# hpcaitech/Open-Sora

Measured on NVIDIA H100. Metric: denoise-steps/sec STDiT3-XL/2 64x32x32 bf16, higher is better.
Workload: dtype bf16

## Files before the change

### open-sora_b200/csrc/attn_sm90.cu

```cuda
#include <stdlib.h>

#include "common.cuh"
#include "stage.cuh"
#include "tiles.cuh"
#include "wgmma.cuh"

namespace osb {

constexpr int kAttnThreads = 256;
constexpr int kKeyBlock = 64;

template <int D>
struct FlashState {
  static constexpr int DP = HeadTileCfg<D>::DP;
  uint32_t q[DP / 16][4];
  float o[DP / 8][4];
  float m[2], l[2];
};

template <int D>
__device__ __forceinline__ void flash_load_q(FlashState<D>& f, uint32_t sq, uint32_t chunk_bytes) {
  using Cfg = HeadTileCfg<D>;
  const int lane = threadIdx.x & 31, warp = threadIdx.x >> 5;
  const int row = warp * 16 + (lane & 15);
#pragma unroll
  for (int kk = 0; kk < Cfg::DP / 16; ++kk)
    ldsm_x4(sq + tile_unit_off<Cfg::MAIN>(row, 2 * kk + (lane >> 4), chunk_bytes), f.q[kk][0], f.q[kk][1], f.q[kk][2], f.q[kk][3]);
#pragma unroll
  for (int j = 0; j < Cfg::DP / 8; ++j) f.o[j][0] = f.o[j][1] = f.o[j][2] = f.o[j][3] = 0.f;
  f.m[0] = f.m[1] = -INFINITY;
  f.l[0] = f.l[1] = 0.f;
}

template <int D, bool kBias = false>
__device__ __forceinline__ void flash_block(FlashState<D>& f, uint32_t sk, uint32_t sv, uint32_t chunk_bytes, int krow0,
                                            int n16, int key0, const int (&lo)[2], const int (&hi)[2], float sc,
                                            const float* bias = nullptr, int boff0 = 0, int boff1 = 0, float bscale = 0.f) {
  using Cfg = HeadTileCfg<D>;
  constexpr int NB = kKeyBlock / 8;
  const int lane = threadIdx.x & 31;
  float s[NB][4];
#pragma unroll
  for (int g = 0; g < kKeyBlock / 16; ++g) {
    s[2 * g][0] = s[2 * g][1] = s[2 * g][2] = s[2 * g][3] = 0.f;
    s[2 * g + 1][0] = s[2 * g + 1][1] = s[2 * g + 1][2] = s[2 * g + 1][3] = 0.f;
    if (g >= n16) continue;
    const int krow = krow0 + g * 16 + (lane & 7) + ((lane >> 4) << 3);
#pragma unroll
    for (int kk = 0; kk < Cfg::DP / 16; ++kk) {
      uint32_t b0, b1, b2, b3;
      ldsm_x4(sk + tile_unit_off<Cfg::MAIN>(krow, 2 * kk + ((lane >> 3) & 1), chunk_bytes), b0, b1, b2, b3);
      mma_bf16_16816(s[2 * g], f.q[kk], b0, b1);
      mma_bf16_16816(s[2 * g + 1], f.q[kk], b2, b3);
// ... 40 lines not shown
    if (g >= n16) continue;
    const uint32_t a[4] = {pack_bf16x2(s[2 * g][0], s[2 * g][1]), pack_bf16x2(s[2 * g][2], s[2 * g][3]),
                           pack_bf16x2(s[2 * g + 1][0], s[2 * g + 1][1]), pack_bf16x2(s[2 * g + 1][2], s[2 * g + 1][3])};
    const int vrow = krow0 + g * 16 + (lane & 7) + (((lane >> 3) & 1) << 3);
#pragma unroll
    for (int dg = 0; dg < Cfg::DP / 16; ++dg) {
      uint32_t b0, b1, b2, b3;
      ldsm_x4_t(sv + tile_unit_off<Cfg::MAIN>(vrow, 2 * dg + (lane >> 4), chunk_bytes), b0, b1, b2, b3);
      mma_bf16_16816(f.o[2 * dg], a, b0, b1);
      mma_bf16_16816(f.o[2 * dg + 1], a, b2, b3);
    }
  }
}

template <int D>
__device__ __forceinline__ void flash_store(FlashState<D>& f, __nv_bfloat16* dst0, __nv_bfloat16* dst1) {
  const int lane = threadIdx.x & 31;
  float inv[2];
#pragma unroll
  for (int i = 0; i < 2; ++i) {
    float l = f.l[i];
    l += __shfl_xor_sync(0xffffffffu, l, 1);
    l += __shfl_xor_sync(0xffffffffu, l, 2);
    inv[i] = l > 0.f ? 1.0f / l : 0.f;
  }
#pragma unroll
  for (int j = 0; j < D / 8; ++j) {
    const int c = 8 * j + 2 * (lane & 3);
    if (dst0) *reinterpret_cast<uint32_t*>(dst0 + c) = pack_bf16x2(f.o[j][0] * inv[0], f.o[j][1] * inv[0]);
    if (dst1) *reinterpret_cast<uint32_t*>(dst1 + c) = pack_bf16x2(f.o[j][2] * inv[1], f.o[j][3] * inv[1]);
  }
}

struct TileAttnParams {
  const uint8_t* q; const uint8_t* k; const uint8_t* v;
  int64_t q_head_stride, kv_head_stride;
  int32_t q_tile_bytes, kv_tile_bytes;
  int64_t items;
  float scale_log2;
  TileSets ts;
};

template <int D>
struct TileAttnSmem {
  static constexpr int kSlot = 128 * HeadTileCfg<D>::ROW_BYTES;
  static constexpr int kStages = D == 128 ? 2 : (D == 72 ? 4 : 5);
  static constexpr int kData = 2 * kSlot + kStages * 2 * kSlot;
  static constexpr int kBytes = 1024 + kData + 8 * (4 + 2 * kStages);
  static_assert(kBytes <= 227 * 1024 && 2 * kBytes > 228 * 1024, "one resident CTA per SM");
};

constexpr int kTileAttnThreads = 384;

template <int D>
__global__ void __launch_bounds__(kTileAttnThreads, 1) attn_tiles_kernel(const TileAttnParams p) {
  using Cfg = HeadTileCfg<D>;
  using Sm = TileAttnSmem<D>;
  constexpr int MAIN = Cfg::MAIN, TAIL = Cfg::TAIL, STAGES = Sm::kStages;
  extern __shared__ uint8_t smem_raw[];
  const uint32_t base = (smem_u32(smem_raw) + 1023u) & ~1023u;
  auto sQ = [&](int b) { return base + (uint32_t)(b * Sm::kSlot); };
  auto sK = [&](int s) { return base + (uint32_t)((2 + 2 * s) * Sm::kSlot); };
  auto sV = [&](int s) { return sK(s) + (uint32_t)Sm::kSlot; };
  const uint32_t bar = base + (uint32_t)Sm::kData;
  auto q_full = [&](int b) { return bar + 8u * b; };
  auto q_empty = [&](int b) { return bar + 16u + 8u * b; };
  auto full_bar = [&](int s) { return bar + 32u + 8u * s; };
  auto empty_bar = [&](int s) { return bar + 32u + 8u * (STAGES + s); };

  const int wg = threadIdx.x >> 7, tid_wg = threadIdx.x & 127;
  const int64_t begin = (int64_t)blockIdx.x * p.items / gridDim.x, end = (int64_t)(blockIdx.x + 1) * p.items / gridDim.x;
  const TileSets& ts = p.ts;
  const int tps = ts.qmap.tps;

  {
    uint4* z = reinterpret_cast<uint4*>(smem_raw + (base - smem_u32(smem_raw)));
    for (int i = threadIdx.x; i < Sm::kData / 16; i += kTileAttnThreads) z[i] = make_uint4(0, 0, 0, 0);
  }
  fence_proxy_async_smem();
  if (threadIdx.x == 0) {
    for (int b = 0; b < 2; ++b) { mbar_init(q_full(b), 1); mbar_init(q_empty(b), 2); }
    for (int s = 0; s < STAGES; ++s) { mbar_init(full_bar(s), 1); mbar_init(empty_bar(s), 2); }
    fence_barrier_init();
  }
  __syncthreads();
  pdl_wait();

  if (wg == 0) {
    asm volatile("setmaxnreg.dec.sync.aligned.u32 40;\n" ::: "memory");
    if (tid_wg == 0) {
      uint32_t kv_it = 0;
      for (int64_t it = begin; it < end; ++it) {
        const uint32_t n = (uint32_t)(it - begin);
        const int64_t hs = it / tps, head = hs / ts.num_sets, set = hs - head * ts.num_sets;
        const int qs = n & 1;
        mbar_wait_notrace(q_empty(qs), ((n >> 1) & 1u) ^ 1u);
        mbar_expect_tx(q_full(qs), (uint32_t)p.q_tile_bytes);
        bulk_load_1d(sQ(qs), p.q + head * p.q_head_stride + (it - head * ts.num_sets * tps) * p.q_tile_bytes,
                     (uint32_t)p.q_tile_bytes, q_full(qs));
        const int nkt = (tile_set_keys(ts, set) + ts.BK - 1) / ts.BK;
        if (it > begin && (it - 1) / tps == hs && nkt <= STAGES) continue;
        const int64_t off = head * p.kv_head_stride + set * ts.nkb * (int64_t)p.kv_tile_bytes;
        for (int t = 0; t < nkt; ++t, ++kv_it) {
          const int s = (int)(kv_it % STAGES);
          mbar_wait_notrace(empty_bar(s), ((kv_it / STAGES) & 1u) ^ 1u);
          mbar_expect_tx(full_bar(s), 2u * (uint32_t)p.kv_tile_bytes);
          bulk_load_1d(sK(s), p.k + off + (int64_t)t * p.kv_tile_bytes, (uint32_t)p.kv_tile_bytes, full_bar(s));
          bulk_load_1d(sV(s), p.v + off + (int64_t)t * p.kv_tile_bytes, (uint32_t)p.kv_tile_bytes, full_bar(s));
        }
      }
      pdl_launch_dependents();
    }
    return;
  }

  asm volatile("setmaxnreg.inc.sync.aligned.u32 232;\n" ::: "memory");
  const int cw = wg - 1;
  const int lane = tid_wg & 31, quad = lane & 3;
  const int r_loc = cw * 64 + (tid_wg >> 5) * 16 + (lane >> 2);
  const float sc = p.scale_log2;
  float s[64], o[MAIN][32], ot[TAIL ? 8 : 1];
#pragma unroll
  for (int i = 0; i < 64; ++i) s[i] = 0.f;
  uint32_t kv_it = 0, kv0 = 0;
  for (int64_t it = begin; it < end; ++it) {
    const uint32_t n = (uint32_t)(it - begin);
    const int64_t hs = it / tps, head = hs / ts.num_sets, set = hs - head * ts.num_sets;
    const int qt = (int)(it - hs * tps), qs = n & 1;
    const int keys = tile_set_keys(ts, set);
    const int nkt = (keys + ts.BK - 1) / ts.BK;
    if (!(it > begin && (it - 1) / tps == hs && nkt <= STAGES)) { kv0 = kv_it; kv_it += nkt; }
    const bool keep = it + 1 < end && (it + 1) / tps == hs && nkt <= STAGES;

    int64_t seq[2];
    int pos[2], lo[2], hi[2];
    bool valid[2];
#pragma unroll
    for (int hh = 0; hh < 2; ++hh) tile_query_row(ts, set, qt, keys, r_loc + 8 * hh, seq[hh], pos[hh], valid[hh], lo[hh], hi[hh]);
#pragma unroll
    for (int c = 0; c < MAIN; ++c)
#pragma unroll
      for (int i = 0; i < 32; ++i) o[c][i] = 0.f;
#pragma unroll
    for (int i = 0; i < (TAIL ? 8 : 1); ++i) ot[i] = 0.f;
    float m[2] = {-INFINITY, -INFINITY}, l[2] = {0.f, 0.f};

    const uint32_t q_chunk = (uint32_t)ts.qmap.TR * 128u, kv_chunk = (uint32_t)ts.BK * 128u;
    const uint32_t qa = sQ(qs) + (uint32_t)(cw * 64 * 128), qa_tail = sQ(qs) + MAIN * q_chunk + (uint32_t)(cw * 8 * 256);
    mbar_wait_notrace(q_full(qs), (n >> 1) & 1u);
    for (int t = 0; t < nkt; ++t) {
      const uint32_t u = kv0 + (uint32_t)t;
      const int st = (int)(u % STAGES);
      mbar_wait_notrace(full_bar(st), (u / STAGES) & 1u);
      const uint32_t ka = sK(st), va = sV(st);
      wgmma_fence_regs(s);
      wgmma_fence();
#pragma unroll
      for (int c = 0; c < MAIN; ++c)
#pragma unroll
        for (int k = 0; k < 4; ++k)
          Wgmma<128>::mma(s, make_sw128_kmajor_desc(qa + c * q_chunk + 32u * k),
                          make_sw128_kmajor_desc(ka + c * kv_chunk + 32u * k), (c | k) ? 1u : 0u);
      if constexpr (TAIL != 0)
        Wgmma<128>::mma(s, make_noswizzle_desc(qa_tail, 128u, 256u), make_noswizzle_desc(ka + MAIN * kv_chunk, 128u, 256u), 1u);
      wgmma_commit();
      wgmma_wait<0>();
      wgmma_fence_regs(s);
      if (t == nkt - 1 && tid_wg == 0) mbar_arrive(q_empty(qs));
      const int slot0 = t * ts.BK;
      const int n16 = ((keys - slot0 < ts.BK ? keys - slot0 : ts.BK) + 15) >> 4;
      float mx[2] = {-INFINITY, -INFINITY};
#pragma unroll
      for (int i = 0; i < 64; ++i) {
        const int hh = (i >> 1) & 1;
        const int col = 8 * (i >> 2) + 2 * quad + (i & 1), key = slot0 + col;
        if (col >= ts.BK || key < lo[hh] || key >= hi[hh]) s[i] = -INFINITY;
        mx[hh] = fmaxf(mx[hh], s[i]);
      }
      float alpha[2], ms[2];
#pragma unroll
      for (int hh = 0; hh < 2; ++hh) {
        mx[hh] = fmaxf(mx[hh], __shfl_xor_sync(0xffffffffu, mx[hh], 1));
        mx[hh] = fmaxf(mx[hh], __shfl_xor_sync(0xffffffffu, mx[hh], 2));
        const float mn = fmaxf(m[hh], mx[hh]);
        alpha[hh] = (mn == -INFINITY) ? 1.f : fast_exp2((m[hh] - mn) * sc);
        ms[hh] = (mn == -INFINITY) ? 0.f : mn * sc;
        m[hh] = mn;
        l[hh] *= alpha[hh];
      }
#pragma unroll
      for (int c = 0; c < MAIN; ++c)
#pragma unroll
        for (int i = 0; i < 32; ++i) o[c][i] *= alpha[(i >> 1) & 1];
      if constexpr (TAIL != 0) {
#pragma unroll
        for (int i = 0; i < 8; ++i) ot[i] *= alpha[(i >> 1) & 1];
      }
      uint32_t pa[8][4];
#pragma unroll
      for (int i = 0; i < 64; ++i) {
        s[i] = (i >> 3) < n16 ? fast_exp2(fmaf(s[i], sc, -ms[(i >> 1) & 1])) : 0.f;
        l[(i >> 1) & 1] += s[i];
      }
#pragma unroll
      for (int g = 0; g < 8; ++g) {
        pa[g][0] = pack_bf16x2(s[8 * g + 0], s[8 * g + 1]);
        pa[g][1] = pack_bf16x2(s[8 * g + 2], s[8 * g + 3]);
        pa[g][2] = pack_bf16x2(s[8 * g + 4], s[8 * g + 5]);
        pa[g][3] = pack_bf16x2(s[8 * g + 6], s[8 * g + 7]);
      }
#pragma unroll
      for (int c = 0; c < MAIN; ++c) wgmma_fence_regs(o[c]);
      if constexpr (TAIL != 0) wgmma_fence_regs(ot);
      wgmma_fence();
#pragma unroll
      for (int g = 0; g < 8; ++g) {
#pragma unroll
        for (int c = 0; c < MAIN; ++c)
          WgmmaRegAT<64>::mma(o[c], pa[g], make_sw128_kmajor_desc(va + c * kv_chunk + 2048u * g), 1u);
        if constexpr (TAIL != 0)
          WgmmaRegAT<16>::mma(ot, pa[g], make_noswizzle_desc(va + MAIN * kv_chunk + 512u * g, 256u, 128u), 1u);
      }
      wgmma_commit();
      wgmma_wait<0>();
#pragma unroll
      for (int c = 0; c < MAIN; ++c) wgmma_fence_regs(o[c]);
      if constexpr (TAIL != 0) wgmma_fence_regs(ot);
#pragma unroll
      for (int g = 0; g < 8; ++g) fence_regs_u32(pa[g]);
      if (!keep && tid_wg == 0) mbar_arrive(empty_bar(st));
    }
    if (nkt == 0 && tid_wg == 0) mbar_arrive(q_empty(qs));

#pragma unroll
    for (int hh = 0; hh < 2; ++hh) {
      float lt = l[hh];
      lt += __shfl_xor_sync(0xffffffffu, lt, 1);
      lt += __shfl_xor_sync(0xffffffffu, lt, 2);
      const float inv = lt > 0.f ? 1.0f / lt : 0.f;
      if (!valid[hh]) continue;
      __nv_bfloat16* dst = tile_out_row(ts, seq[hh], pos[hh]) + head * D + 2 * quad;
#pragma unroll
      for (int c = 0; c < MAIN; ++c)
#pragma unroll
        for (int j = 0; j < 8; ++j)
          *reinterpret_cast<uint32_t*>(dst + 64 * c + 8 * j) = pack_bf16x2(o[c][4 * j + 2 * hh] * inv, o[c][4 * j + 2 * hh + 1] * inv);
      if constexpr (TAIL != 0)
        *reinterpret_cast<uint32_t*>(dst + 64 * MAIN) = pack_bf16x2(ot[2 * hh] * inv, ot[2 * hh + 1] * inv);
    }
  }
}

template <int D>
static int attn_tiles_launch(TileAttnParams& p, int H, cudaStream_t stream) {
  using Cfg = HeadTileCfg<D>;
  p.q_tile_bytes = p.ts.qmap.TR * Cfg::ROW_BYTES;
  p.kv_tile_bytes = p.ts.BK * Cfg::ROW_BYTES;
  p.items = (int64_t)H * p.ts.num_sets * p.ts.qmap.tps;
  if (p.items >= (1ll << 31)) { set_error("osb_attn_tiles: problem too large (%lld work items)", (long long)p.items); return OSB_ERR_UNSUPPORTED; }
  const int64_t grid = p.items < sm_count() ? p.items : sm_count();
  cudaLaunchAttribute attr[2];
  cudaLaunchConfig_t cfg = launch_config(dim3((unsigned)grid), dim3(kTileAttnThreads), TileAttnSmem<D>::kBytes, stream, attr);
  OSB_CHECK_CUDA(cudaLaunchKernelEx(&cfg, attn_tiles_kernel<D>, p));
  count_launch();
  return OSB_OK;
}

struct AttnParams {
  const __nv_bfloat16* q; const __nv_bfloat16* k; const __nv_bfloat16* v; __nv_bfloat16* out;
  int64_t q_ld, k_ld, v_ld, out_ld;
  int64_t num_seqs, seqs_per_batch;
  int64_t q_bs, q_ss, q_ts, k_bs, k_ss, k_ts;
  int32_t Lq, Lk;
  const int32_t* kv_lens;
  const __nv_bfloat16* qw; const __nv_bfloat16* kw;
  const __nv_bfloat16* qw2; const __nv_bfloat16* kw2;
  int32_t norm_split;
  float eps;
  const float* cos; const float* sin;
  int32_t rope_half;
  float scale_log2;
  int32_t G;
  int32_t tiles_per_seq;
  const float* bias;
  int64_t bias_hs;
  float scale;
};

template <int D>
__device__ __forceinline__ void stage_row(uint4 (&raw)[HeadTileCfg<D>::U], bool norm, float eps, const __nv_bfloat16* w,
                                          const float* cosr, const float* sinr, bool rope_half, uint8_t* tile,
                                          uint32_t chunk_bytes, int row) {
  using Cfg = HeadTileCfg<D>;
  constexpr int U = Cfg::U;
  norm_rope_row<D, U>(raw, norm, eps, w, cosr, sinr, rope_half);
#pragma unroll
  for (int u = 0; u < Cfg::UP; ++u)
    *reinterpret_cast<uint4*>(tile + tile_unit_off<Cfg::MAIN>(row, u, chunk_bytes)) = u < U ? raw[u] : make_uint4(0, 0, 0, 0);
}

template <int D, bool kBias>
__global__ void __launch_bounds__(kAttnThreads, 1) attn_short_kernel(const AttnParams p) {
  using Cfg = HeadTileCfg<D>;
  constexpr int U = Cfg::U;
  extern __shared__ __align__(1024) uint8_t smem[];
  uint8_t* sQ = smem;
  uint8_t* sK = smem + 128 * Cfg::ROW_BYTES;
  uint8_t* sV = sK + kKeyBlock * Cfg::ROW_BYTES;
  const int tid = threadIdx.x, lane = tid & 31, warp = tid >> 5;
  const int64_t unit = blockIdx.x;
  const int h = blockIdx.y;

  int64_t seq0;
  int qt = 0;
  if (p.G > 1) seq0 = unit * p.G;
  else { seq0 = unit / p.tiles_per_seq; qt = (int)(unit - seq0 * p.tiles_per_seq); }
// ... 70 lines not shown
      const int slot = k0 + s;
      const int kg = slot / p.Lk, ktok = slot - kg * p.Lk;
      const int64_t kseq = seq0 + kg;
      const bool ok = slot < nkeys && kseq < p.num_seqs;
      int64_t krow = 0;
      if (ok) krow = row_of(kseq, ktok, p.k_bs, p.k_ss, p.k_ts);
      uint4 t[U];
      {
        const uint4* ks = reinterpret_cast<const uint4*>(p.k + krow * p.k_ld + (int64_t)h * D);
#pragma unroll
        for (int u = 0; u < U; ++u) t[u] = ok ? __ldg(ks + u) : make_uint4(0, 0, 0, 0);
        const __nv_bfloat16* w = (p.kw2 != nullptr && ktok >= p.norm_split) ? p.kw2 : p.kw;
        const bool rope = ok && p.cos != nullptr;
        stage_row<D>(t, ok && p.kw != nullptr, p.eps, w, rope ? p.cos + (int64_t)ktok * (D / 2) : nullptr,
                     rope ? p.sin + (int64_t)ktok * (D / 2) : nullptr, p.rope_half, sK, kKeyBlock * 128u, s);
      }
      {
        const uint4* vs = reinterpret_cast<const uint4*>(p.v + krow * p.v_ld + (int64_t)h * D);
#pragma unroll
        for (int u = 0; u < U; ++u) t[u] = ok ? __ldg(vs + u) : make_uint4(0, 0, 0, 0);
        stage_row<D>(t, false, 0.f, nullptr, nullptr, nullptr, false, sV, kKeyBlock * 128u, s);
      }
    }
    __syncthreads();
    const int n = nkeys - k0 < kKeyBlock ? nkeys - k0 : kKeyBlock;
    if constexpr (kBias)
      flash_block<D, true>(f, smem_u32(sK), smem_u32(sV), kKeyBlock * 128u, 0, (n + 15) >> 4, k0, lo, hi, sc, bh, boff[0],
                           boff[1], p.scale);
    else
      flash_block<D>(f, smem_u32(sK), smem_u32(sV), kKeyBlock * 128u, 0, (n + 15) >> 4, k0, lo, hi, sc);
    __syncthreads();
  }
  pdl_launch_dependents();
  flash_store<D>(f, dst[0], dst[1]);
}

template <int D, bool kBias = false>
static int attn_short_launch(const AttnParams& p, int64_t units, int H, cudaStream_t stream) {
  using Cfg = HeadTileCfg<D>;
  const int smem = (128 + 2 * kKeyBlock) * Cfg::ROW_BYTES;
  cudaLaunchAttribute attr[2];
  cudaLaunchConfig_t cfg = launch_config(dim3((unsigned)units, (unsigned)H), dim3(kAttnThreads), smem, stream, attr);
  OSB_CHECK_CUDA(cudaLaunchKernelEx(&cfg, attn_short_kernel<D, kBias>, p));
  count_launch();
  return OSB_OK;
}

int attn_init() {
  constexpr int kMax = 200 * 1024;
  OSB_CHECK_CUDA(cudaFuncSetAttribute(attn_short_kernel<64, false>, cudaFuncAttributeMaxDynamicSharedMemorySize, kMax));
  OSB_CHECK_CUDA(cudaFuncSetAttribute(attn_short_kernel<72, false>, cudaFuncAttributeMaxDynamicSharedMemorySize, kMax));
  OSB_CHECK_CUDA(cudaFuncSetAttribute(attn_short_kernel<128, false>, cudaFuncAttributeMaxDynamicSharedMemorySize, kMax));
  OSB_CHECK_CUDA(cudaFuncSetAttribute(attn_short_kernel<64, true>, cudaFuncAttributeMaxDynamicSharedMemorySize, kMax));
  OSB_CHECK_CUDA(cudaFuncSetAttribute(attn_tiles_kernel<64>, cudaFuncAttributeMaxDynamicSharedMemorySize, TileAttnSmem<64>::kBytes));
  OSB_CHECK_CUDA(cudaFuncSetAttribute(attn_tiles_kernel<72>, cudaFuncAttributeMaxDynamicSharedMemorySize, TileAttnSmem<72>::kBytes));
  OSB_CHECK_CUDA(cudaFuncSetAttribute(attn_tiles_kernel<128>, cudaFuncAttributeMaxDynamicSharedMemorySize, TileAttnSmem<128>::kBytes));
  return OSB_OK;
}

int make_tile_map(TileMap* dst, const osb_tile_map& m, const char* who) {
  OSB_REQUIRE(m.mode == 0 || m.mode == 1, "%s: unknown tile map mode %d", who, m.mode);
  OSB_REQUIRE(m.L > 0 && m.G >= 1 && m.tile_rows > 0 && m.tile_rows <= 128 && m.tile_rows % 8 == 0,
              "%s: bad tile map (L %d G %d rows %d)", who, m.L, m.G, m.tile_rows);
  OSB_REQUIRE(m.G == 1 ? (m.tps == (m.L + m.tile_rows - 1) / m.tile_rows) : (m.G * m.L <= m.tile_rows && m.tps == 1),
              "%s: tile map inconsistent (L %d G %d tps %d rows %d)", who, m.L, m.G, m.tps, m.tile_rows);
  OSB_REQUIRE(m.mode == 0 || (m.S > 0 && m.T == m.L), "%s: temporal map needs S > 0 and T == L", who);
  dst->mode = m.mode; dst->L = m.L; dst->S = m.S; dst->T = m.T; dst->G = m.G; dst->tps = m.tps; dst->TR = m.tile_rows;
  return OSB_OK;
}

int make_tile_sets(TileSets* dst, const osb_attn_tiles_args* a, const char* who) {
  OSB_REQUIRE(a->out || a->out_scatter, "%s: null tensor", who);
  const int rc = make_tile_map(&dst->qmap, a->q_map, who);
  if (rc) return rc;
  const int G = a->q_map.G;
  OSB_REQUIRE(a->kv_tile_rows >= 16 && a->kv_tile_rows <= 128 && a->kv_tile_rows % 16 == 0,
              "%s: key tiles must have 16..128 rows in multiples of 16, got %d", who, a->kv_tile_rows);
  OSB_REQUIRE(a->Lk > 0 && a->kv_tiles_per_set >= 1 && (int64_t)a->kv_tiles_per_set * a->kv_tile_rows >= (int64_t)(G > 1 ? G : 1) * a->Lk,
              "%s: %d key tiles of %d rows cannot hold %d keys", who, a->kv_tiles_per_set, a->kv_tile_rows, a->Lk);
  OSB_REQUIRE(G == 1 || (a->kv_tiles_per_set == 1), "%s: packed sequences use one key tile per set", who);
  OSB_REQUIRE(a->num_seqs > 0 && a->num_heads > 0, "%s: empty problem", who);
  OSB_REQUIRE(a->out_ld % 8 == 0 && (reinterpret_cast<uintptr_t>(a->out) & 15) == 0, "%s: out must be 16-byte aligned", who);
  dst->BK = a->kv_tile_rows; dst->nkb = a->kv_tiles_per_set; dst->Lk = a->Lk;
  dst->num_seqs = a->num_seqs;
  dst->num_sets = G > 1 ? (a->num_seqs + G - 1) / G : a->num_seqs;
  dst->kv_lens = a->kv_lens;
  dst->out = static_cast<__nv_bfloat16*>(a->out);
  dst->out_ld = a->out_ld;
  return make_row_scatter(&dst->out_sc, a->out_scatter, a->num_seqs * a->q_map.L, who);
}

int check_attn_short_args(const osb_attn_short_args* a, const char* who) {
  OSB_REQUIRE(a != nullptr, "%s: null args", who);
  OSB_REQUIRE(a->q && a->k && a->v && a->out, "%s: null tensor", who);
  OSB_REQUIRE(a->Lq > 0 && a->Lk > 0 && a->num_seqs > 0 && a->num_heads > 0, "%s: empty problem", who);
  OSB_REQUIRE(a->seqs_per_batch > 0, "%s: seqs_per_batch must be positive", who);
  OSB_REQUIRE((a->q_ld % 8) == 0 && (a->k_ld % 8) == 0 && (a->v_ld % 8) == 0 && (a->out_ld % 8) == 0,
              "%s: leading dimensions must be multiples of 8 elements", who);
  OSB_REQUIRE(((reinterpret_cast<uintptr_t>(a->q) | reinterpret_cast<uintptr_t>(a->k) |
                reinterpret_cast<uintptr_t>(a->v) | reinterpret_cast<uintptr_t>(a->out)) & 15) == 0,
              "%s: tensors must be 16-byte aligned", who);
  OSB_REQUIRE((a->q_norm_w == nullptr) == (a->k_norm_w == nullptr), "%s: q/k norm weights must come together", who);
  OSB_REQUIRE((a->rope_cos == nullptr) == (a->rope_sin == nullptr), "%s: rope cos/sin must come together", who);
  OSB_REQUIRE((a->q_norm_w2 == nullptr) == (a->k_norm_w2 == nullptr) && (a->q_norm_w2 == nullptr || a->q_norm_w != nullptr),
              "%s: the second norm weight pair needs the first", who);
  OSB_REQUIRE(a->rope_cos == nullptr || ((reinterpret_cast<uintptr_t>(a->rope_cos) | reinterpret_cast<uintptr_t>(a->rope_sin)) & 15) == 0,
              "%s: rope tables must be 16-byte aligned", who);
  return OSB_OK;
}

}

extern "C" int64_t osb_head_tiles_per_head(const osb_tile_map* m, int64_t rows) {
  if (m == nullptr || m->L <= 0 || m->tile_rows <= 0) return -1;
  const int64_t seqs = rows / m->L;
  if (m->G > 1) return (seqs + m->G - 1) / m->G;
  return seqs * m->tps;
}

extern "C" int osb_attn_tiles(const osb_attn_tiles_args* a, void* stream) {
  using namespace osb;
  if (!initialised()) { set_error("osb_init() has not been called"); return OSB_ERR_NOT_INIT; }
  OSB_REQUIRE(a != nullptr, "osb_attn_tiles: null args");
  OSB_REQUIRE(a->q_tiles && a->k_tiles && a->v_tiles, "osb_attn_tiles: null tensor");
  const int D = a->head_dim;
  OSB_REQUIRE(D == 64 || D == 72 || D == 128, "osb_attn_tiles: head_dim %d not built (64, 72, 128)", D);
  OSB_REQUIRE(((reinterpret_cast<uintptr_t>(a->q_tiles) | reinterpret_cast<uintptr_t>(a->k_tiles) | reinterpret_cast<uintptr_t>(a->v_tiles)) & 15) == 0 &&
              a->q_head_stride % 16 == 0 && a->kv_head_stride % 16 == 0, "osb_attn_tiles: tile buffers must be 16-byte aligned");

  TileAttnParams p = {};
  const int rc = make_tile_sets(&p.ts, a, "osb_attn_tiles");
  if (rc) return rc;
  p.q = static_cast<const uint8_t*>(a->q_tiles);
  p.k = static_cast<const uint8_t*>(a->k_tiles);
  p.v = static_cast<const uint8_t*>(a->v_tiles);
  p.q_head_stride = a->q_head_stride; p.kv_head_stride = a->kv_head_stride;
  p.scale_log2 = a->softmax_scale * 1.4426950408889634f;
  cudaStream_t s = static_cast<cudaStream_t>(stream);
  if (D == 64) return attn_tiles_launch<64>(p, a->num_heads, s);
  if (D == 72) return attn_tiles_launch<72>(p, a->num_heads, s);
  return attn_tiles_launch<128>(p, a->num_heads, s);
}

static int attn_short_entry(const osb_attn_short_args* a, const float* bias, int64_t bias_head_stride, void* stream) {
  using namespace osb;
  if (!initialised()) { set_error("osb_init() has not been called"); return OSB_ERR_NOT_INIT; }
  const int rc = check_attn_short_args(a, "osb_attn_short");
  if (rc) return rc;
  const int D = a->head_dim;
  OSB_REQUIRE(D == 64 || D == 72 || D == 128, "osb_attn_short: head_dim %d not built (64, 72, 128)", D);

  AttnParams p;
  p.q = static_cast<const __nv_bfloat16*>(a->q);
  p.k = static_cast<const __nv_bfloat16*>(a->k);
  p.v = static_cast<const __nv_bfloat16*>(a->v);
  p.out = static_cast<__nv_bfloat16*>(a->out);
  p.q_ld = a->q_ld; p.k_ld = a->k_ld; p.v_ld = a->v_ld; p.out_ld = a->out_ld;
  p.num_seqs = a->num_seqs; p.seqs_per_batch = a->seqs_per_batch;
  p.q_bs = a->q_batch_stride; p.q_ss = a->q_seq_stride; p.q_ts = a->q_tok_stride;
  p.k_bs = a->k_batch_stride; p.k_ss = a->k_seq_stride; p.k_ts = a->k_tok_stride;
  p.Lq = a->Lq; p.Lk = a->Lk; p.kv_lens = a->kv_lens;
  p.qw = static_cast<const __nv_bfloat16*>(a->q_norm_w);
  p.kw = static_cast<const __nv_bfloat16*>(a->k_norm_w);
  p.qw2 = static_cast<const __nv_bfloat16*>(a->q_norm_w2);
  p.kw2 = static_cast<const __nv_bfloat16*>(a->k_norm_w2);
  p.norm_split = a->norm_split;
  p.eps = a->norm_eps;
  p.cos = a->rope_cos; p.sin = a->rope_sin;
  p.rope_half = a->rope_cos != nullptr && a->rope_half ? 1 : 0;
  OSB_REQUIRE(!p.rope_half || (D % 16 == 0), "osb_attn_short: rotate-half RoPE needs head_dim %% 16 == 0");
  p.scale_log2 = a->softmax_scale * 1.4426950408889634f;
  int64_t units;
  if (a->Lq >= 128) {
    p.G = 1;
    p.tiles_per_seq = (a->Lq + 127) / 128;
    units = a->num_seqs * p.tiles_per_seq;
  } else {
    p.G = 128 / a->Lq;
    p.tiles_per_seq = 1;
    units = (a->num_seqs + p.G - 1) / p.G;
  }
  OSB_REQUIRE((int64_t)p.G * a->Lk < (1ll << 31), "osb_attn_short: too many keys per query tile");
  OSB_REQUIRE(units <= 0x7fffffff && a->num_heads <= 65535, "osb_attn_short: grid too large");
  cudaStream_t s = static_cast<cudaStream_t>(stream);
  p.bias = bias;
  p.bias_hs = bias_head_stride;
  p.scale = a->softmax_scale;
  if (bias != nullptr) {
    OSB_REQUIRE(D == 64, "osb_attn_short_bias: head_dim %d not built (64)", D);
    OSB_REQUIRE(bias_head_stride >= 0, "osb_attn_short_bias: negative bias_head_stride");
    p.scale_log2 = 1.4426950408889634f;
    return attn_short_launch<64, true>(p, units, a->num_heads, s);
  }
  if (D == 64) return attn_short_launch<64>(p, units, a->num_heads, s);
// ... 11 lines not shown
```

### open-sora_b200/csrc/wgmma.cuh

```cuda
#pragma once

#include <stdint.h>

namespace osb {

template <int N>
struct Wgmma;

template <>
struct Wgmma<64> {
  static constexpr int kRegs = 32;
  __device__ __forceinline__ static void mma(float (&d)[32], uint64_t da, uint64_t db, uint32_t accumulate) {
    asm volatile(
        "{\n\t.reg .pred p;\n\tsetp.ne.b32 p, %34, 0;\n\t"
        "wgmma.mma_async.sync.aligned.m64n64k16.f32.bf16.bf16 "
        "{%0, %1, %2, %3, %4, %5, %6, %7, %8, %9, %10, %11, %12, %13, %14, %15, %16, %17, %18, %19, %20, %21, %22, %23, %24, %25, %26, %27, %28, %29, %30, %31}, "
        "%32, %33, p, 1, 1, 0, 0;\n\t}\n"
        : "+f"(d[0]), "+f"(d[1]), "+f"(d[2]), "+f"(d[3]), "+f"(d[4]), "+f"(d[5]), "+f"(d[6]), "+f"(d[7]),
        "+f"(d[8]), "+f"(d[9]), "+f"(d[10]), "+f"(d[11]), "+f"(d[12]), "+f"(d[13]), "+f"(d[14]), "+f"(d[15]),
        "+f"(d[16]), "+f"(d[17]), "+f"(d[18]), "+f"(d[19]), "+f"(d[20]), "+f"(d[21]), "+f"(d[22]), "+f"(d[23]),
        "+f"(d[24]), "+f"(d[25]), "+f"(d[26]), "+f"(d[27]), "+f"(d[28]), "+f"(d[29]), "+f"(d[30]), "+f"(d[31])
        : "l"(da), "l"(db), "r"(accumulate));
  }
};

template <>
struct Wgmma<128> {
  static constexpr int kRegs = 64;
  __device__ __forceinline__ static void mma(float (&d)[64], uint64_t da, uint64_t db, uint32_t accumulate) {
    asm volatile(
        "{\n\t.reg .pred p;\n\tsetp.ne.b32 p, %66, 0;\n\t"
        "wgmma.mma_async.sync.aligned.m64n128k16.f32.bf16.bf16 "
        "{%0, %1, %2, %3, %4, %5, %6, %7, %8, %9, %10, %11, %12, %13, %14, %15, %16, %17, %18, %19, %20, %21, %22, %23, %24, %25, %26, %27, %28, %29, %30, %31, %32, %33, %34, %35, %36, %37, %38, %39, %40, %41, %42, %43, %44, %45, %46, %47, %48, %49, %50, %51, %52, %53, %54, %55, %56, %57, %58, %59, %60, %61, %62, %63}, "
        "%64, %65, p, 1, 1, 0, 0;\n\t}\n"
        : "+f"(d[0]), "+f"(d[1]), "+f"(d[2]), "+f"(d[3]), "+f"(d[4]), "+f"(d[5]), "+f"(d[6]), "+f"(d[7]),
        "+f"(d[8]), "+f"(d[9]), "+f"(d[10]), "+f"(d[11]), "+f"(d[12]), "+f"(d[13]), "+f"(d[14]), "+f"(d[15]),
        "+f"(d[16]), "+f"(d[17]), "+f"(d[18]), "+f"(d[19]), "+f"(d[20]), "+f"(d[21]), "+f"(d[22]), "+f"(d[23]),
        "+f"(d[24]), "+f"(d[25]), "+f"(d[26]), "+f"(d[27]), "+f"(d[28]), "+f"(d[29]), "+f"(d[30]), "+f"(d[31]),
        "+f"(d[32]), "+f"(d[33]), "+f"(d[34]), "+f"(d[35]), "+f"(d[36]), "+f"(d[37]), "+f"(d[38]), "+f"(d[39]),
        "+f"(d[40]), "+f"(d[41]), "+f"(d[42]), "+f"(d[43]), "+f"(d[44]), "+f"(d[45]), "+f"(d[46]), "+f"(d[47]),
        "+f"(d[48]), "+f"(d[49]), "+f"(d[50]), "+f"(d[51]), "+f"(d[52]), "+f"(d[53]), "+f"(d[54]), "+f"(d[55]),
        "+f"(d[56]), "+f"(d[57]), "+f"(d[58]), "+f"(d[59]), "+f"(d[60]), "+f"(d[61]), "+f"(d[62]), "+f"(d[63])
        : "l"(da), "l"(db), "r"(accumulate));
  }
};

template <>
struct Wgmma<144> {
  static constexpr int kRegs = 72;
  __device__ __forceinline__ static void mma(float (&d)[72], uint64_t da, uint64_t db, uint32_t accumulate) {
    asm volatile(
        "{\n\t.reg .pred p;\n\tsetp.ne.b32 p, %74, 0;\n\t"
        "wgmma.mma_async.sync.aligned.m64n144k16.f32.bf16.bf16 "
        "{%0, %1, %2, %3, %4, %5, %6, %7, %8, %9, %10, %11, %12, %13, %14, %15, %16, %17, %18, %19, %20, %21, %22, %23, %24, %25, %26, %27, %28, %29, %30, %31, %32, %33, %34, %35, %36, %37, %38, %39, %40, %41, %42, %43, %44, %45, %46, %47, %48, %49, %50, %51, %52, %53, %54, %55, %56, %57, %58, %59, %60, %61, %62, %63, %64, %65, %66, %67, %68, %69, %70, %71}, "
        "%72, %73, p, 1, 1, 0, 0;\n\t}\n"
        : "+f"(d[0]), "+f"(d[1]), "+f"(d[2]), "+f"(d[3]), "+f"(d[4]), "+f"(d[5]), "+f"(d[6]), "+f"(d[7]),
        "+f"(d[8]), "+f"(d[9]), "+f"(d[10]), "+f"(d[11]), "+f"(d[12]), "+f"(d[13]), "+f"(d[14]), "+f"(d[15]),
        "+f"(d[16]), "+f"(d[17]), "+f"(d[18]), "+f"(d[19]), "+f"(d[20]), "+f"(d[21]), "+f"(d[22]), "+f"(d[23]),
        "+f"(d[24]), "+f"(d[25]), "+f"(d[26]), "+f"(d[27]), "+f"(d[28]), "+f"(d[29]), "+f"(d[30]), "+f"(d[31]),
        "+f"(d[32]), "+f"(d[33]), "+f"(d[34]), "+f"(d[35]), "+f"(d[36]), "+f"(d[37]), "+f"(d[38]), "+f"(d[39]),
// ... 264 lines not shown
```

Before: 11.96.

## Narrow attention tile MMAs to per-warpgroup key windows in packed-tile attention

Adds a windowed variant of the tile attention kernel. Each consumer warpgroup computes the key range its query rows can attend to, then runs a narrower wgmma (N=16/32/64/128) over only that slice of the key tile. Masking is skipped when the whole slice lies inside a single window, and the output epilogue is changed to shuffle values into 16-byte stores. The variant is chosen at launch when the tile sets have multiple groups per tile, variable kv lengths, or unaligned key lengths. This cuts wasted MMA and exp work on packed short sequences, at the cost of more template instantiations and branching.

```diff
diff --git a/open-sora_b200/csrc/attn_sm90.cu b/open-sora_b200/csrc/attn_sm90.cu
--- a/open-sora_b200/csrc/attn_sm90.cu
+++ b/open-sora_b200/csrc/attn_sm90.cu
@@ -1,4 +1,6 @@
 #include <stdlib.h>
+
+#include <type_traits>
 
 #include "common.cuh"
 #include "stage.cuh"
@@ -145,7 +147,7 @@
 
 constexpr int kTileAttnThreads = 384;
 
-template <int D>
+template <int D, bool kWindows>
 __global__ void __launch_bounds__(kTileAttnThreads, 1) attn_tiles_kernel(const TileAttnParams p) {
   using Cfg = HeadTileCfg<D>;
   using Sm = TileAttnSmem<D>;
@@ -212,9 +214,7 @@
   const int lane = tid_wg & 31, quad = lane & 3;
   const int r_loc = cw * 64 + (tid_wg >> 5) * 16 + (lane >> 2);
   const float sc = p.scale_log2;
-  float s[64], o[MAIN][32], ot[TAIL ? 8 : 1];
-#pragma unroll
-  for (int i = 0; i < 64; ++i) s[i] = 0.f;
+  float o[MAIN][32], ot[TAIL ? 8 : 1];
   uint32_t kv_it = 0, kv0 = 0;
   for (int64_t it = begin; it < end; ++it) {
     const uint32_t n = (uint32_t)(it - begin);
@@ -238,6 +238,21 @@
     for (int i = 0; i < (TAIL ? 8 : 1); ++i) ot[i] = 0.f;
     float m[2] = {-INFINITY, -INFINITY}, l[2] = {0.f, 0.f};
 
+    int wlo = 0, whi = keys;
+    bool single = true;
+    if constexpr (kWindows) {
+      whi = 0;
+      if (ts.qmap.G > 1) {
+        const int g0 = cw * 64 / ts.qmap.L;
+        const int64_t last = min((int64_t)ts.qmap.G, ts.num_seqs - set * ts.qmap.G) - 1;
+        const int g1 = (int)min((int64_t)((cw * 64 + 63) / ts.qmap.L), last);
+        if (g0 <= g1) { wlo = g0 * ts.Lk; whi = (g1 + 1) * ts.Lk; }
+        single = g0 == g1;
+      } else if (cw * 64 < ts.qmap.TR && qt * ts.qmap.TR + cw * 64 < ts.qmap.L) {
+        whi = keys;
+      }
+    }
+
     const uint32_t q_chunk = (uint32_t)ts.qmap.TR * 128u, kv_chunk = (uint32_t)ts.BK * 128u;
     const uint32_t qa = sQ(qs) + (uint32_t)(cw * 64 * 128), qa_tail = sQ(qs) + MAIN * q_chunk + (uint32_t)(cw * 8 * 256);
     mbar_wait_notrace(q_full(qs), (n >> 1) & 1u);
@@ -246,105 +261,158 @@
       const int st = (int)(u % STAGES);
       mbar_wait_notrace(full_bar(st), (u / STAGES) & 1u);
       const uint32_t ka = sK(st), va = sV(st);
-      wgmma_fence_regs(s);
-      wgmma_fence();
-#pragma unroll
-      for (int c = 0; c < MAIN; ++c)
-#pragma unroll
-        for (int k = 0; k < 4; ++k)
-          Wgmma<128>::mma(s, make_sw128_kmajor_desc(qa + c * q_chunk + 32u * k),
-                          make_sw128_kmajor_desc(ka + c * kv_chunk + 32u * k), (c | k) ? 1u : 0u);
-      if constexpr (TAIL != 0)
-        Wgmma<128>::mma(s, make_noswizzle_desc(qa_tail, 128u, 256u), make_noswizzle_desc(ka + MAIN * kv_chunk, 128u, 256u), 1u);
-      wgmma_commit();
-      wgmma_wait<0>();
-      wgmma_fence_regs(s);
-      if (t == nkt - 1 && tid_wg == 0) mbar_arrive(q_empty(qs));
+      const bool last = t == nkt - 1;
       const int slot0 = t * ts.BK;
-      const int n16 = ((keys - slot0 < ts.BK ? keys - slot0 : ts.BK) + 15) >> 4;
-      float mx[2] = {-INFINITY, -INFINITY};
-#pragma unroll
-      for (int i = 0; i < 64; ++i) {
-        const int hh = (i >> 1) & 1;
-        const int col = 8 * (i >> 2) + 2 * quad + (i & 1), key = slot0 + col;
-        if (col >= ts.BK || key < lo[hh] || key >= hi[hh]) s[i] = -INFINITY;
-        mx[hh] = fmaxf(mx[hh], s[i]);
-      }
-      float alpha[2], ms[2];
-#pragma unroll
-      for (int hh = 0; hh < 2; ++hh) {
-        mx[hh] = fmaxf(mx[hh], __shfl_xor_sync(0xffffffffu, mx[hh], 1));
-        mx[hh] = fmaxf(mx[hh], __shfl_xor_sync(0xffffffffu, mx[hh], 2));
-        const float mn = fmaxf(m[hh], mx[hh]);
-        alpha[hh] = (mn == -INFINITY) ? 1.f : fast_exp2((m[hh] - mn) * sc);
-        ms[hh] = (mn == -INFINITY) ? 0.f : mn * sc;
-        m[hh] = mn;
-        l[hh] *= alpha[hh];
-      }
-#pragma unroll
-      for (int c = 0; c < MAIN; ++c)
-#pragma unroll
-        for (int i = 0; i < 32; ++i) o[c][i] *= alpha[(i >> 1) & 1];
-      if constexpr (TAIL != 0) {
-#pragma unroll
-        for (int i = 0; i < 8; ++i) ot[i] *= alpha[(i >> 1) & 1];
-      }
-      uint32_t pa[8][4];
-#pragma unroll
-      for (int i = 0; i < 64; ++i) {
-        s[i] = (i >> 3) < n16 ? fast_exp2(fmaf(s[i], sc, -ms[(i >> 1) & 1])) : 0.f;
-        l[(i >> 1) & 1] += s[i];
-      }
-#pragma unroll
-      for (int g = 0; g < 8; ++g) {
-        pa[g][0] = pack_bf16x2(s[8 * g + 0], s[8 * g + 1]);
-        pa[g][1] = pack_bf16x2(s[8 * g + 2], s[8 * g + 3]);
-        pa[g][2] = pack_bf16x2(s[8 * g + 4], s[8 * g + 5]);
-        pa[g][3] = pack_bf16x2(s[8 * g + 6], s[8 * g + 7]);
-      }
-#pragma unroll
-      for (int c = 0; c < MAIN; ++c) wgmma_fence_regs(o[c]);
-      if constexpr (TAIL != 0) wgmma_fence_regs(ot);
-      wgmma_fence();
-#pragma unroll
-      for (int g = 0; g < 8; ++g) {
+      const int w0 = wlo - slot0 > 0 ? wlo - slot0 : 0;
+      const int w1 = whi - slot0 < ts.BK ? whi - slot0 : ts.BK;
+
+      auto tile_step = [&](auto kn, int off) {
+        constexpr int KN = decltype(kn)::value;
+        float sk[KN / 2];
+#pragma unroll
+        for (int i = 0; i < KN / 2; ++i) sk[i] = 0.f;
+        const uint32_t kb = ka + (uint32_t)off * 128u;
+        wgmma_fence_regs(sk);
+        wgmma_fence();
 #pragma unroll
         for (int c = 0; c < MAIN; ++c)
-          WgmmaRegAT<64>::mma(o[c], pa[g], make_sw128_kmajor_desc(va + c * kv_chunk + 2048u * g), 1u);
+#pragma unroll
+          for (int k = 0; k < 4; ++k)
+            Wgmma<KN>::mma(sk, make_sw128_kmajor_desc(qa + c * q_chunk + 32u * k),
+                           make_sw128_kmajor_desc(kb + c * kv_chunk + 32u * k), (c | k) ? 1u : 0u);
         if constexpr (TAIL != 0)
-          WgmmaRegAT<16>::mma(ot, pa[g], make_noswizzle_desc(va + MAIN * kv_chunk + 512u * g, 256u, 128u), 1u);
-      }
-      wgmma_commit();
-      wgmma_wait<0>();
-#pragma unroll
-      for (int c = 0; c < MAIN; ++c) wgmma_fence_regs(o[c]);
-      if constexpr (TAIL != 0) wgmma_fence_regs(ot);
-#pragma unroll
-      for (int g = 0; g < 8; ++g) fence_regs_u32(pa[g]);
+          Wgmma<KN>::mma(sk, make_noswizzle_desc(qa_tail, 128u, 256u),
+                         make_noswizzle_desc(ka + MAIN * kv_chunk + (uint32_t)off * 32u, 128u, 256u), 1u);
+        wgmma_commit();
+        wgmma_wait<0>();
+        wgmma_fence_regs(sk);
+        if (last && tid_wg == 0) mbar_arrive(q_empty(qs));
+        const int n16 = (w1 - off + 15) >> 4;
+        float mx[2] = {-INFINITY, -INFINITY};
+        if (single && off >= w0 && off + KN <= w1) {
+#pragma unroll
+          for (int i = 0; i < KN / 2; ++i) mx[(i >> 1) & 1] = fmaxf(mx[(i >> 1) & 1], sk[i]);
+        } else {
+#pragma unroll
+          for (int i = 0; i < KN / 2; ++i) {
+            const int hh = (i >> 1) & 1;
+            const int col = off + 8 * (i >> 2) + 2 * quad + (i & 1), key = slot0 + col;
+            if (col >= ts.BK || key < lo[hh] || key >= hi[hh]) sk[i] = -INFINITY;
+            mx[hh] = fmaxf(mx[hh], sk[i]);
+          }
+        }
+        float alpha[2], ms[2];
+#pragma unroll
+        for (int hh = 0; hh < 2; ++hh) {
+          mx[hh] = fmaxf(mx[hh], __shfl_xor_sync(0xffffffffu, mx[hh], 1));
+          mx[hh] = fmaxf(mx[hh], __shfl_xor_sync(0xffffffffu, mx[hh], 2));
+          const float mn = fmaxf(m[hh], mx[hh]);
+          alpha[hh] = (mn == -INFINITY) ? 1.f : fast_exp2((m[hh] - mn) * sc);
+          ms[hh] = (mn == -INFINITY) ? 0.f : mn * sc;
+          m[hh] = mn;
+          l[hh] *= alpha[hh];
+        }
+#pragma unroll
+        for (int c = 0; c < MAIN; ++c)
+#pragma unroll
+          for (int i = 0; i < 32; ++i) o[c][i] *= alpha[(i >> 1) & 1];
+        if constexpr (TAIL != 0) {
+#pragma unroll
+          for (int i = 0; i < 8; ++i) ot[i] *= alpha[(i >> 1) & 1];
+        }
+        uint32_t pa[KN / 16][4];
+#pragma unroll
+        for (int i = 0; i < KN / 2; ++i) {
+          sk[i] = (i >> 3) < n16 ? fast_exp2(fmaf(sk[i], sc, -ms[(i >> 1) & 1])) : 0.f;
+          l[(i >> 1) & 1] += sk[i];
+        }
+#pragma unroll
+        for (int g = 0; g < KN / 16; ++g) {
+          pa[g][0] = pack_bf16x2(sk[8 * g + 0], sk[8 * g + 1]);
+          pa[g][1] = pack_bf16x2(sk[8 * g + 2], sk[8 * g + 3]);
+          pa[g][2] = pack_bf16x2(sk[8 * g + 4], sk[8 * g + 5]);
+          pa[g][3] = pack_bf16x2(sk[8 * g + 6], sk[8 * g + 7]);
+        }
+        const uint32_t vb = va + (uint32_t)off * 128u;
+#pragma unroll
+        for (int c = 0; c < MAIN; ++c) wgmma_fence_regs(o[c]);
+        if constexpr (TAIL != 0) wgmma_fence_regs(ot);
+        wgmma_fence();
+#pragma unroll
+        for (int g = 0; g < KN / 16; ++g) {
+#pragma unroll
+          for (int c = 0; c < MAIN; ++c)
+            WgmmaRegAT<64>::mma(o[c], pa[g], make_sw128_kmajor_desc(vb + c * kv_chunk + 2048u * g), 1u);
+          if constexpr (TAIL != 0)
+            WgmmaRegAT<16>::mma(ot, pa[g], make_noswizzle_desc(va + MAIN * kv_chunk + (uint32_t)off * 32u + 512u * g, 256u, 128u), 1u);
+        }
+        wgmma_commit();
+        wgmma_wait<0>();
+#pragma unroll
+        for (int c = 0; c < MAIN; ++c) wgmma_fence_regs(o[c]);
+        if constexpr (TAIL != 0) wgmma_fence_regs(ot);
+#pragma unroll
+        for (int g = 0; g < KN / 16; ++g) fence_regs_u32(pa[g]);
+      };
+      if constexpr (!kWindows) {
+        tile_step(std::integral_constant<int, 128>{}, 0);
+      } else if (w1 > w0) {
+        const int off = w0 >= 64 ? 64 : 0, span = w1 - off;
+        if (span > 64) tile_step(std::integral_constant<int, 128>{}, 0);
+        else if (span > 32) tile_step(std::integral_constant<int, 64>{}, off);
+        else if (span > 16) tile_step(std::integral_constant<int, 32>{}, off);
+        else tile_step(std::integral_constant<int, 16>{}, off);
+      } else if (last && tid_wg == 0) {
+        mbar_arrive(q_empty(qs));
+      }
       if (!keep && tid_wg == 0) mbar_arrive(empty_bar(st));
     }
     if (nkt == 0 && tid_wg == 0) mbar_arrive(q_empty(qs));
 
+    const bool odd = (lane & 1) != 0, high = (lane & 2) != 0;
 #pragma unroll
     for (int hh = 0; hh < 2; ++hh) {
       float lt = l[hh];
       lt += __shfl_xor_sync(0xffffffffu, lt, 1);
       lt += __shfl_xor_sync(0xffffffffu, lt, 2);
       const float inv = lt > 0.f ? 1.0f / lt : 0.f;
-      if (!valid[hh]) continue;
-      __nv_bfloat16* dst = tile_out_row(ts, seq[hh], pos[hh]) + head * D + 2 * quad;
-#pragma unroll
-      for (int c = 0; c < MAIN; ++c)
-#pragma unroll
-        for (int j = 0; j < 8; ++j)
-          *reinterpret_cast<uint32_t*>(dst + 64 * c + 8 * j) = pack_bf16x2(o[c][4 * j + 2 * hh] * inv, o[c][4 * j + 2 * hh + 1] * inv);
-      if constexpr (TAIL != 0)
-        *reinterpret_cast<uint32_t*>(dst + 64 * MAIN) = pack_bf16x2(ot[2 * hh] * inv, ot[2 * hh + 1] * inv);
-    }
-  }
-}
-
-template <int D>
+      if constexpr (!kWindows) {
+        if (!valid[hh]) continue;
+        __nv_bfloat16* dst = tile_out_row(ts, seq[hh], pos[hh]) + head * D + 2 * quad;
+#pragma unroll
+        for (int c = 0; c < MAIN; ++c)
+#pragma unroll
+          for (int j = 0; j < 8; ++j)
+            *reinterpret_cast<uint32_t*>(dst + 64 * c + 8 * j) = pack_bf16x2(o[c][4 * j + 2 * hh] * inv, o[c][4 * j + 2 * hh + 1] * inv);
+        if constexpr (TAIL != 0)
+          *reinterpret_cast<uint32_t*>(dst + 64 * MAIN) = pack_bf16x2(ot[2 * hh] * inv, ot[2 * hh + 1] * inv);
+        continue;
+      }
+      __nv_bfloat16* dst = valid[hh] ? tile_out_row(ts, seq[hh], pos[hh]) + head * D : nullptr;
+#pragma unroll
+      for (int c = 0; c < MAIN; ++c) {
+#pragma unroll
+        for (int j0 = 0; j0 < 8; j0 += 4) {
+          const float* x = &o[c][4 * j0 + 2 * hh];
+          uint32_t u0 = pack_bf16x2(x[0] * inv, x[1] * inv), u1 = pack_bf16x2(x[4] * inv, x[5] * inv);
+          uint32_t u2 = pack_bf16x2(x[8] * inv, x[9] * inv), u3 = pack_bf16x2(x[12] * inv, x[13] * inv);
+          uint32_t s0 = __shfl_xor_sync(0xffffffffu, odd ? u0 : u1, 1);
+          uint32_t s1 = __shfl_xor_sync(0xffffffffu, odd ? u2 : u3, 1);
+          if (odd) { u0 = s0; u2 = s1; } else { u1 = s0; u3 = s1; }
+          s0 = __shfl_xor_sync(0xffffffffu, high ? u0 : u2, 2);
+          s1 = __shfl_xor_sync(0xffffffffu, high ? u1 : u3, 2);
+          if (high) { u0 = s0; u1 = s1; } else { u2 = s0; u3 = s1; }
+          if (dst) *reinterpret_cast<uint4*>(dst + 64 * c + 8 * (j0 + quad)) = make_uint4(u0, u1, u2, u3);
+        }
+      }
+      if constexpr (TAIL != 0) {
+        if (dst) *reinterpret_cast<uint32_t*>(dst + 64 * MAIN + 2 * quad) = pack_bf16x2(ot[2 * hh] * inv, ot[2 * hh + 1] * inv);
+      }
+    }
+  }
+}
+
+template <int D, bool kWindows>
 static int attn_tiles_launch(TileAttnParams& p, int H, cudaStream_t stream) {
   using Cfg = HeadTileCfg<D>;
   p.q_tile_bytes = p.ts.qmap.TR * Cfg::ROW_BYTES;
@@ -354,7 +422,7 @@
   const int64_t grid = p.items < sm_count() ? p.items : sm_count();
   cudaLaunchAttribute attr[2];
   cudaLaunchConfig_t cfg = launch_config(dim3((unsigned)grid), dim3(kTileAttnThreads), TileAttnSmem<D>::kBytes, stream, attr);
-  OSB_CHECK_CUDA(cudaLaunchKernelEx(&cfg, attn_tiles_kernel<D>, p));
+  OSB_CHECK_CUDA(cudaLaunchKernelEx(&cfg, attn_tiles_kernel<D, kWindows>, p));
   count_launch();
   return OSB_OK;
 }
@@ -531,9 +599,12 @@
   OSB_CHECK_CUDA(cudaFuncSetAttribute(attn_short_kernel<72, false>, cudaFuncAttributeMaxDynamicSharedMemorySize, kMax));
   OSB_CHECK_CUDA(cudaFuncSetAttribute(attn_short_kernel<128, false>, cudaFuncAttributeMaxDynamicSharedMemorySize, kMax));
   OSB_CHECK_CUDA(cudaFuncSetAttribute(attn_short_kernel<64, true>, cudaFuncAttributeMaxDynamicSharedMemorySize, kMax));
-  OSB_CHECK_CUDA(cudaFuncSetAttribute(attn_tiles_kernel<64>, cudaFuncAttributeMaxDynamicSharedMemorySize, TileAttnSmem<64>::kBytes));
-  OSB_CHECK_CUDA(cudaFuncSetAttribute(attn_tiles_kernel<72>, cudaFuncAttributeMaxDynamicSharedMemorySize, TileAttnSmem<72>::kBytes));
-  OSB_CHECK_CUDA(cudaFuncSetAttribute(attn_tiles_kernel<128>, cudaFuncAttributeMaxDynamicSharedMemorySize, TileAttnSmem<128>::kBytes));
+  for (const void* k : {(const void*)attn_tiles_kernel<64, false>, (const void*)attn_tiles_kernel<64, true>})
+    OSB_CHECK_CUDA(cudaFuncSetAttribute(k, cudaFuncAttributeMaxDynamicSharedMemorySize, TileAttnSmem<64>::kBytes));
+  for (const void* k : {(const void*)attn_tiles_kernel<72, false>, (const void*)attn_tiles_kernel<72, true>})
+    OSB_CHECK_CUDA(cudaFuncSetAttribute(k, cudaFuncAttributeMaxDynamicSharedMemorySize, TileAttnSmem<72>::kBytes));
+  for (const void* k : {(const void*)attn_tiles_kernel<128, false>, (const void*)attn_tiles_kernel<128, true>})
+    OSB_CHECK_CUDA(cudaFuncSetAttribute(k, cudaFuncAttributeMaxDynamicSharedMemorySize, TileAttnSmem<128>::kBytes));
   return OSB_OK;
 }
 
@@ -616,9 +687,15 @@
   p.q_head_stride = a->q_head_stride; p.kv_head_stride = a->kv_head_stride;
   p.scale_log2 = a->softmax_scale * 1.4426950408889634f;
   cudaStream_t s = static_cast<cudaStream_t>(stream);
-  if (D == 64) return attn_tiles_launch<64>(p, a->num_heads, s);
-  if (D == 72) return attn_tiles_launch<72>(p, a->num_heads, s);
-  return attn_tiles_launch<128>(p, a->num_heads, s);
+  const bool windows = p.ts.qmap.G > 1 || p.ts.kv_lens != nullptr || p.ts.BK != 128 || p.ts.Lk % 128 != 0;
+  if (windows) {
+    if (D == 64) return attn_tiles_launch<64, true>(p, a->num_heads, s);
+    if (D == 72) return attn_tiles_launch<72, true>(p, a->num_heads, s);
+    return attn_tiles_launch<128, true>(p, a->num_heads, s);
+  }
+  if (D == 64) return attn_tiles_launch<64, false>(p, a->num_heads, s);
+  if (D == 72) return attn_tiles_launch<72, false>(p, a->num_heads, s);
+  return attn_tiles_launch<128, false>(p, a->num_heads, s);
 }
 
 static int attn_short_entry(const osb_attn_short_args* a, const float* bias, int64_t bias_head_stride, void* stream) {
diff --git a/open-sora_b200/csrc/wgmma.cuh b/open-sora_b200/csrc/wgmma.cuh
--- a/open-sora_b200/csrc/wgmma.cuh
+++ b/open-sora_b200/csrc/wgmma.cuh
@@ -6,6 +6,35 @@
 
 template <int N>
 struct Wgmma;
+
+template <>
+struct Wgmma<16> {
+  static constexpr int kRegs = 8;
+  __device__ __forceinline__ static void mma(float (&d)[8], uint64_t da, uint64_t db, uint32_t accumulate) {
+    asm volatile(
+        "{\n\t.reg .pred p;\n\tsetp.ne.b32 p, %10, 0;\n\t"
+        "wgmma.mma_async.sync.aligned.m64n16k16.f32.bf16.bf16 "
+        "{%0, %1, %2, %3, %4, %5, %6, %7}, "
+        "%8, %9, p, 1, 1, 0, 0;\n\t}\n"
+        : "+f"(d[0]), "+f"(d[1]), "+f"(d[2]), "+f"(d[3]), "+f"(d[4]), "+f"(d[5]), "+f"(d[6]), "+f"(d[7])
+        : "l"(da), "l"(db), "r"(accumulate));
+  }
+};
+
+template <>
+struct Wgmma<32> {
+  static constexpr int kRegs = 16;
+  __device__ __forceinline__ static void mma(float (&d)[16], uint64_t da, uint64_t db, uint32_t accumulate) {
+    asm volatile(
+        "{\n\t.reg .pred p;\n\tsetp.ne.b32 p, %18, 0;\n\t"
+        "wgmma.mma_async.sync.aligned.m64n32k16.f32.bf16.bf16 "
+        "{%0, %1, %2, %3, %4, %5, %6, %7, %8, %9, %10, %11, %12, %13, %14, %15}, "
+        "%16, %17, p, 1, 1, 0, 0;\n\t}\n"
+        : "+f"(d[0]), "+f"(d[1]), "+f"(d[2]), "+f"(d[3]), "+f"(d[4]), "+f"(d[5]), "+f"(d[6]), "+f"(d[7]),
+        "+f"(d[8]), "+f"(d[9]), "+f"(d[10]), "+f"(d[11]), "+f"(d[12]), "+f"(d[13]), "+f"(d[14]), "+f"(d[15])
+        : "l"(da), "l"(db), "r"(accumulate));
+  }
+};
 
 template <>
 struct Wgmma<64> {
```

Result: faster. 12.32, median of 6 (+3.0%).
